# Yuki-Kumon/deepmatching_stereo_matching

Hardware: AMD Instinct MI355X
Metric: correlation-volume G-voxels/sec + ms/stereo-pair @1/8 GPU, 1024^2 d=128 (higher is better)
Workload: dtype u8->i32/f32/f64; 1 GPU; C3: 1024x1024 pair, 8x8 tiles of S=128, ws=5, full pyramid + sub-pixel + cal_map + stitch; tile=128, tiles_per_pair=64, window_size=5, pyramid_levels=full, parallelism=pairs sharded 1-way, streams=2, level_stream=False, stats_stream=False, pair_priority=normal, chain_levels=True

## Files before the change

deepmatching_stereo_matching_amd/_lib.py:

```python

import ctypes
import os
import re

import torch

HERE = os.path.dirname(os.path.abspath(__file__))
LIB_PATH = os.environ.get('DM_LIB_PATH') or os.path.join(HERE, 'libdmstereo.so')
HEADER = os.path.join(os.path.dirname(HERE), 'include', 'dmstereo.h')

DM_OK, DM_ERR_ARG, DM_ERR_SHAPE, DM_ERR_UNSUPPORTED, DM_ERR_HIP = 0, -1, -2, -3, -4
DM_VOLUME_F16, DM_VOLUME_MINMAX_KNOWN = 1, 2
DM_POW_F32, DM_POW_Q4, DM_POW_K, DM_POW_FULL, DM_POW_Q4G, DM_POW_KG = 0, 1, 2, 3, 4, 5
DM_TM_CCOEFF, DM_TM_CCOEFF_NORMED = 4, 5
METHODS = {'cv2.TM_CCOEFF_NORMED': DM_TM_CCOEFF_NORMED, 'cv2.TM_CCOEFF': DM_TM_CCOEFF}
CAL_MODES = {'elevation': 0, 'elevation2': 1, 'distance': 2}
DM_GS_FWD4, DM_GS_BWD4, DM_GS_BILAT = 0, 1, 2
DM_MERGE_LAST, DM_MERGE_CENTER, DM_MERGE_FEATHER, DM_MERGE_MEDIAN = 0, 1, 2, 3
MERGE_RULES = {'last': DM_MERGE_LAST, 'center': DM_MERGE_CENTER, 'feather': DM_MERGE_FEATHER,
               'median': DM_MERGE_MEDIAN}
DM_MERGE_MAX_CAND = 64
DM_BILAT_FILL, DM_BILAT_GUIDE_U8 = 1, 2
DM_MEDIAN_FILL = 1

# ... 2 lines not shown
    pass


class DmError(RuntimeError):
    pass


class DmTiles(ctypes.Structure):
    _fields_ = [('d_img1', ctypes.c_void_p), ('d_img2', ctypes.c_void_p),
                ('pitch1', ctypes.c_int32), ('pitch2', ctypes.c_int32),
                ('d_origins', ctypes.c_void_p), ('T', ctypes.c_int32),
                ('h0', ctypes.c_int32), ('w0', ctypes.c_int32),
                ('ws', ctypes.c_int32), ('method', ctypes.c_int32)]


_P = ctypes.c_void_p
_I = ctypes.c_int32
_TP = ctypes.POINTER(DmTiles)
SIGNATURES = {
    'dm_abi_version': ([], ctypes.c_int),
    'dm_last_error': ([], ctypes.c_char_p),
    'dm_build_config': ([], ctypes.c_char_p),
    'dm_stats_bytes': ([_TP], ctypes.c_size_t),
    'dm_corr_stats': ([_TP, _P, _P], ctypes.c_int),
    'dm_corr_level1': ([_TP, _P, _P, _P], ctypes.c_int),
    'dm_corr_level12': ([_TP, _P, _P, _P, _P], ctypes.c_int),
    'dm_corr_volume': ([_TP, _P, _P, _P], ctypes.c_int),
    'dm_corr_volume_f16': ([_TP, _P, _P, _P], ctypes.c_int),
    'dm_corr_volume_ex': ([_TP, _P, _I, _P, _P], ctypes.c_int),
    'dm_rectify_f16': ([_P, ctypes.c_size_t, _P, _P], ctypes.c_int),
    'dm_rectify': ([_P, ctypes.c_size_t, _P, _P], ctypes.c_int),
    'dm_rectify64': ([_P, ctypes.c_size_t, _P, _P], ctypes.c_int),
    'dm_pow14_variant': ([_I, _P, ctypes.c_size_t, _P, _P], ctypes.c_int),
    'dm_aggregate': ([_P, _I, _I, _I, _I, _P, _P], ctypes.c_int),
    'dm_match': ([_TP, _P, ctypes.POINTER(ctypes.c_void_p), _I, _I, _I, _I, _I, _I, _I, _I,
                  _P, _P, _P], ctypes.c_int),
    'dm_subpix_map': ([_P, _I, _I, _I, _I, _I, _P, _P], ctypes.c_int),
    'dm_subpix_map_tiles': ([_TP, _P, _I, _I, _P, _P], ctypes.c_int),
    'dm_sub_pix_cal': ([_P, _P, _I, _I, _I, ctypes.c_double, _P, _P], ctypes.c_int),
    'dm_cal_map': ([_P, _I, _I, _I, _I, _P, _P], ctypes.c_int),
    'dm_gs_schedule': ([_I, _I, _I, _I, _I, _I, _P, _P, ctypes.POINTER(ctypes.c_int32)], ctypes.c_int),
    'dm_image_threshold': ([_P, ctypes.c_size_t, ctypes.c_double, ctypes.c_double, _P, _P], ctypes.c_int),
    'dm_optimize_loop': ([_P, _P, _I, _I, _I, _I, _I, _I, _I, ctypes.c_double, _P, _P, _I, _P, _P, _I,
                          _P, _P, _P], ctypes.c_int),
    'dm_make_weight': ([_P, _I, _I, _I, _I, _I, ctypes.c_double, ctypes.c_double, _P, _P, _P], ctypes.c_int),
    'dm_opt_loop_bilateral': ([_P, _P, _P, _P, _I, _I, _I, _I, _I, _I, _I, _I, _P, _P, _I, _P, _P, _P],
                              ctypes.c_int),
    'dm_stitch': ([_P, _I, _I, _I, _I, _I, _I, ctypes.POINTER(ctypes.c_int32), _I, _P, _P, _P],
                  ctypes.c_int),
    'dm_seq_sum': ([_P, ctypes.c_int64, _P, _P], ctypes.c_int),
    'dm_fb_check': ([_P, _P, _I, _I, _I, ctypes.c_double, _P, _P, _P], ctypes.c_int),
    'dm_stitch_fb': ([_P, _P, _I, _I, _I, _I, _I, _I, ctypes.POINTER(ctypes.c_int32), _I, ctypes.c_double,
                      _P, _P, _P, _P], ctypes.c_int),
    'dm_stitch_merge': ([_P, _P, _I, _I, _I, _I, _I, _I, ctypes.POINTER(ctypes.c_int32), _I, ctypes.c_double,
                         _I, _I, _P, _P, _P, _P, _P, _P], ctypes.c_int),
    'dm_fill_bytes': ([_I, _I, _I], ctypes.c_size_t),
    'dm_fill_holes': ([_P, _I, _I, _I, _I, _P, _P, _P, _P], ctypes.c_int),
    'dm_speckle_bytes': ([_I, _I, _I], ctypes.c_size_t),
    'dm_filter_speckles': ([_P, _I, _I, _I, _I, ctypes.c_double, _P, _P, _P, _P, _P, _P], ctypes.c_int),
    'dm_bilateral_bytes': ([_I, _I, _I], ctypes.c_size_t),
    'dm_bilateral_filter': ([_P, _P, _I, _I, _I, _I, _I, ctypes.c_double, ctypes.c_double, _I, _I, _P, _P, _P, _P],
                            ctypes.c_int),
    'dm_median_bytes': ([_I, _I, _I], ctypes.c_size_t),
    'dm_median_filter': ([_P, _P, _I, _I, _I, _I, _I, _I, _I, _I, _P, _P, _P, _P], ctypes.c_int),
}

# ... 56 lines not shown
```

deepmatching_stereo_matching_amd/csrc/dm_kernels.hip:

```cpp
#include <hip/hip_runtime.h>

#include <stdarg.h>
#include <stdlib.h>
#include <stdio.h>
#include <string.h>

#include <type_traits>

#include "../../include/dmstereo.h"
#include "dm_pow.h"

__constant__ double c_pow_tab[DM_POW_NT * 3] = DM_POW_TAB_INIT;
__constant__ double c_pow_g[10] = DM_POW_G_INIT;
__constant__ double c_powf_c[DM_POWF_NT] = DM_POWF_C_INIT;
__constant__ double c_powf_p[DM_POWF_NT * 2] = DM_POWF_P_INIT;
__constant__ double c_powf_g[(1 - DM_POWF_EMIN) * 2] = DM_POWF_G_INIT;

#ifdef DM_TAIL_PRIO
#define DM_TAIL_ENTRY() __builtin_amdgcn_s_setprio(3)
#else
#define DM_TAIL_ENTRY() ((void)0)
#endif

__device__ __forceinline__ double pow14(double x)
// ... 1100 lines not shown

static int mfq_nw(const dm_tiles *b)
{
    const int G = b->w0 / 16;
    const bool g4 = b->ws * b->ws <= 25 && G % 4 == 0 && (G / 4 == 1 || G / 4 == 2 || G / 4 == 4);
    if (g4) return G / 4;
    return G / 2 < 8 ? G / 2 : 8;
}

static bool volume_ls_shape(const dm_tiles *b)
{
    return mf16_eligible(b) && b->ws <= 5 && (b->h0 % 4) == 0 && ((size_t)(b->h0 / 4) * (b->w0 / 4)) % 8 == 0;
}


#ifndef DM_S1
#define DM_S1 1
#endif
static bool strip_shape(const dm_tiles *b)
{
    if (!DM_S1 || !mf16_eligible(b) || b->ws > 5) return false;
    const int G = b->w0 / 16;
    return G % 4 == 0 && (G / 4 == 1 || G / 4 == 2 || G / 4 == 4);
}

#ifndef DM_S2
#define DM_S2 5
#endif
static bool strip2_shape(const dm_tiles *b)
{
    return strip_shape(b) && ((DM_S2 >> (b->w0 == 64 ? 0 : b->w0 == 128 ? 1 : 2)) & 1);
}

static size_t strip_bytes(const dm_tiles *b)
{
    const size_t rows = (size_t)b->T * (b->h0 / 2);
    return rows * (b->w0 / 32) * 1024 + rows * b->w0 * 16;
}

static void strip_views(const dm_tiles *b, void *d_stats, dm_v4i **Bs, dm_v4i **Ss)
{
    const size_t extra = mf16_extra_bytes(b);
    char *base = (char *)d_stats + align256(base_stats_bytes(b)) + align256(extra) +
                 (volume_ls_shape(b) ? align256(extra) : 0);
    *Bs = (dm_v4i *)base;
    *Ss = (dm_v4i *)(base + (size_t)b->T * (b->h0 / 2) * (b->w0 / 32) * 1024);
}

static void mfma_views2(const dm_tiles *b, void *d_stats, dm_v4i **Bw, int2 **QS)
{
    const int G = b->w0 / 16;
    char *base = (char *)d_stats + align256(base_stats_bytes(b)) + align256(mf16_extra_bytes(b));
    *Bw = (dm_v4i *)base;
    *QS = (int2 *)(base + (size_t)b->T * b->h0 * G * 1024);
}

static void mfma_views(const dm_tiles *b, void *d_stats, dm_v4i **Bw, int2 **QS)
{
    const int G = b->w0 / 16, KS = (b->ws * b->ws + 63) / 64;
    char *base = (char *)d_stats + align256(base_stats_bytes(b));
    *Bw = (dm_v4i *)base;
    *QS = (int2 *)(base + (size_t)b->T * b->h0 * G * KS * 1024);
}

static inline unsigned nblk(size_t n, unsigned bs)
{
// ... 156 lines not shown
static int launch_mfq_t(const dm_tiles *b, Stats s, const dm_v4i *Bw, const int2 *QS, double *L1, double *L2,
                        hipStream_t st, const dm_v4i *Bs, const dm_v4i *Ss)
{
    const int KS = (b->ws * b->ws + 63) / 64, NW = mfq_nw(b), GW = b->w0 / 16 / NW;
    const unsigned grid = (unsigned)(b->T * (b->h0 / 4) * (b->w0 / 4));
    const Geo gg = make_geo(b);
    constexpr bool CL = L2F;
    if (KS == 1 && GW == 4 && NW == 4) {
        constexpr int NBc = DM_C5_NB;
        const size_t bpt = (size_t)(b->h0 / 4) * (b->w0 / 4);
        if (bpt % NBc) return fail(DM_ERR_UNSUPPORTED, "cell blocks per tile not a multiple of %d (fill_ptab: a workgroup in one tile)", NBc);
        if (Bs && (DM_S2 & 4)) k_level12_strip<4, NBc, L2F, CL, 4><<<grid / NBc, 64 * 4 * NBc, 0, st>>>(gg, s, L1, L2, Bs, Ss);
        else if (Bs) k_level1_mfq<1, 4, 4 * NBc, 4, L2F, YF, NBc, CL, YF><<<grid / NBc, 64 * 4 * NBc, 0, st>>>(gg, s, Bw, QS, L1, L2, Bs, Ss);
        else k_level1_mfq<1, 4, 4 * NBc, 4, L2F, YF, NBc, CL><<<grid / NBc, 64 * 4 * NBc, 0, st>>>(gg, s, Bw, QS, L1, L2);
        HIP_TRY(hipGetLastError());
        return DM_OK;
    }
    if (KS == 1 && GW == 4 && NW == 1) {
        constexpr int NBc = DM_C2_NB;
        const size_t bpt = (size_t)(b->h0 / 4) * (b->w0 / 4);
        if (bpt % NBc) return fail(DM_ERR_UNSUPPORTED, "cell blocks per tile not a multiple of %d (fill_ptab: a workgroup in one tile)", NBc);
        if (Bs && (DM_S2 & 1)) k_level12_strip<1, NBc, L2F, CL, 4><<<grid / NBc, 64 * NBc, 0, st>>>(gg, s, L1, L2, Bs, Ss);
        else if (Bs) k_level1_mfq<1, 4, NBc, 4, L2F, YF, NBc, CL, YF><<<grid / NBc, 64 * NBc, 0, st>>>(gg, s, Bw, QS, L1, L2, Bs, Ss);
        else k_level1_mfq<1, 4, NBc, 4, L2F, YF, NBc, CL><<<grid / NBc, 64 * NBc, 0, st>>>(gg, s, Bw, QS, L1, L2);
        HIP_TRY(hipGetLastError());
        return DM_OK;
    }
    if (KS == 1 && GW == 4 && NW == 2) {
        constexpr int NBc = DM_C3_NB;
        const size_t bpt = (size_t)(b->h0 / 4) * (b->w0 / 4);
        if (bpt % NBc) return fail(DM_ERR_UNSUPPORTED, "cell blocks per tile not a multiple of %d (fill_ptab: a workgroup in one tile)", NBc);
        if (Bs && (DM_S2 & 2)) k_level12_strip<2, NBc, L2F, CL, DM_C3_MW><<<grid / NBc, 64 * 2 * NBc, 0, st>>>(gg, s, L1, L2, Bs, Ss);
        else if (prune_c3<L2F && YF>(gg, s, L1, L2, Bw, QS, Bs, Ss, grid / NBc, st)) {}
        else if (Bs) k_level1_mfq<1, 4, 2 * NBc, DM_C3_MINW, L2F, YF, NBc, CL, YF><<<grid / NBc, 64 * 2 * NBc, 0, st>>>(gg, s, Bw, QS, L1, L2, Bs, Ss);
        else k_level1_mfq<1, 4, 2 * NBc, 4, L2F, YF, NBc, CL><<<grid / NBc, 64 * 2 * NBc, 0, st>>>(gg, s, Bw, QS, L1, L2);
        HIP_TRY(hipGetLastError());
        return DM_OK;
    }
#define DM_MQ(KS_, GW_, NW_) if (KS == KS_ && GW == GW_ && NW == NW_) { k_level1_mfq<KS_, GW_, NW_, 5, L2F, YF><<<grid, 64 * NW_, 0, st>>>(gg, s, Bw, QS, L1, L2); HIP_TRY(hipGetLastError()); return DM_OK; }
    DM_MQ(1, 2, 1) DM_MQ(1, 2, 2) DM_MQ(1, 2, 4) DM_MQ(1, 2, 8)
    if constexpr (!YF) {
        DM_MQ(2, 2, 1) DM_MQ(2, 2, 2) DM_MQ(2, 2, 4) DM_MQ(2, 2, 8)
        DM_MQ(3, 2, 1) DM_MQ(3, 2, 2) DM_MQ(3, 2, 4) DM_MQ(3, 2, 8)
        DM_MQ(4, 2, 1) DM_MQ(4, 2, 2) DM_MQ(4, 2, 4) DM_MQ(4, 2, 8)
    }
#undef DM_MQ
    return fail(DM_ERR_UNSUPPORTED, "no column-split instance for KS=%d GW=%d NW=%d", KS, GW, NW);
}

template <bool L2F>
static int launch_mfq(const dm_tiles *b, void *d_stats, double *L1, double *L2, hipStream_t st)
{
    dm_v4i *Bw;
    int2 *QS;
    mfma_views(b, d_stats, &Bw, &QS);
    const Stats s = stats_view(d_stats, b->T, b->h0 * b->w0);
    dm_v4i *Bs = nullptr, *Ss = nullptr;
    if (strip_shape(b)) strip_views(b, d_stats, &Bs, &Ss);
    if (b->ws <= 5) return launch_mfq_t<L2F, true>(b, s, Bw, QS, L1, L2, st, Bs, Ss);
    return launch_mfq_t<L2F, false>(b, s, Bw, QS, L1, L2, st, nullptr, nullptr);
}

#ifndef DM_VL_H_TR
#define DM_VL_H_TR 2
#endif
#ifndef DM_VL_H_NT
// ... 99 lines not shown
    }
#define DM_VL(G_) if (G == G_) { k_volume_ls<G_, 8, true, OT><<<grid, 64 * 8, 0, st>>>(gg, s, Bw, QS, out, have_mm, Bs, Ss); HIP_TRY(hipGetLastError()); return DM_OK; }
    DM_VL(2) DM_VL(4) DM_VL(8) DM_VL(16)
#undef DM_VL
    return DM_ERR_UNSUPPORTED;
}

template <typename OT>
static int launch_volume_mfq(const dm_tiles *b, void *d_stats, const Stats &s, OT *out, hipStream_t st)
{
    dm_v4i *Bw;
    int2 *QS;
    mfma_views(b, d_stats, &Bw, &QS);
    const int KS = (b->ws * b->ws + 63) / 64, GW = b->w0 / 16 / mfq_nw(b);
    const size_t waves = (size_t)b->T * (b->h0 / 4) * (b->w0 / 4);
    const unsigned vgrid = (unsigned)((waves + 3) / 4);
    const bool lds = b->w0 <= 128;
    const Geo gg = make_geo(b);
#define DM_VQ(KS_, LS_) if (KS == KS_ && GW == 2 && lds == LS_) { k_volume_mfq<KS_, 2, false, true, LS_, OT><<<vgrid, 256, 0, st>>>(gg, s, Bw, QS, out); HIP_TRY(hipGetLastError()); return DM_OK; }
    DM_VQ(1, true) DM_VQ(1, false) DM_VQ(2, true) DM_VQ(2, false)
    DM_VQ(3, true) DM_VQ(3, false) DM_VQ(4, true) DM_VQ(4, false)
#undef DM_VQ
    return DM_ERR_UNSUPPORTED;
}

extern "C" {

int dm_abi_version(void) { return 110; }

#define DM_STR2(x) #x
#define DM_STR(x) DM_STR2(x)
const char *dm_build_config(void)
{
    return "S1=" DM_STR(DM_S1) " S2=" DM_STR(DM_S2) " PRUNE=" DM_STR(DM_PRUNE) " STRIP_WAVESYNC=" DM_STR(DM_STRIP_WAVESYNC) " VS1=" DM_STR(DM_VS1) " VS1_LDS=" DM_STR(DM_VS1_LDS) " XCD_MAP=" DM_STR(DM_XCD_MAP) " C2_NB=" DM_STR(DM_C2_NB) " C3_NB=" DM_STR(DM_C3_NB) " C3_MW=" DM_STR(DM_C3_MW) " C3_MINW=" DM_STR(DM_C3_MINW) " C5_NB=" DM_STR(DM_C5_NB)
           " VL_H_TR=" DM_STR(DM_VL_H_TR) " VL_H_NT=" DM_STR(DM_VL_H_NT) " VL_H_NW=" DM_STR(DM_VL_H_NW)
           " VL_H2_TR=" DM_STR(DM_VL_H2_TR) " VL_H2_NW=" DM_STR(DM_VL_H2_NW) " VL_F2_TR=" DM_STR(DM_VL_F2_TR)
           " VL_F2_MW=" DM_STR(DM_VL_F2_MW) " VL_HS_NW=" DM_STR(DM_VL_HS_NW) " VL_HS_TR=" DM_STR(DM_VL_HS_TR) " VL_F_NW=" DM_STR(DM_VL_F_NW)
           " VL_F_TR=" DM_STR(DM_VL_F_TR) " VL_F_MW=" DM_STR(DM_VL_F_MW) " VL_F_NT=" DM_STR(DM_VL_F_NT);
}

#if DM_CLOCK_STAMP
int dm_diag_clock_stamps(unsigned long long *host, int nwg)
{
    if (nwg < 0 || nwg > 65536) return fail(DM_ERR_ARG, "nwg %d outside 0 .. 65536", nwg);
    HIP_TRY(hipMemcpyFromSymbol(host, HIP_SYMBOL(dm_clock_stamps), (size_t)nwg * 4 * sizeof(unsigned long long)));
    return DM_OK;
}
#endif

const char *dm_last_error(void) { return g_err; }

size_t dm_stats_bytes(const dm_tiles *b)
{
    if (!b) return 0;
    size_t n = base_stats_bytes(b), extra = 0;
    if (b->ws >= 1 && b->ws <= 15 && b->T > 0 && b->h0 > 0 && b->w0 > 0 && mf16_eligible(b))
        extra = mf16_extra_bytes(b);
    if (!extra) return n;
    size_t tot = align256(n) + align256(extra);
    if (volume_ls_shape(b)) tot += align256(extra);
    if (strip_shape(b)) tot += strip_bytes(b);
    return tot;
}

int dm_corr_stats(const dm_tiles *b, void *d_stats, void *stream)
{
    int rc = check_tiles(b);
    if (rc) return rc;
    if (!d_stats) return fail(DM_ERR_ARG, "null stats workspace");
    const int P = b->h0 * b->w0;
    dim3 grid(nblk(P, 256), b->T);
    k_stats<<<grid, 256, 0, (hipStream_t)stream>>>(make_geo(b), stats_view(d_stats, b->T, P));
    HIP_TRY(hipGetLastError());
    const int var = level1_variant(b);
    if (var) {
        dm_v4i *Bw;
        int2 *QS;
        mfma_views(b, d_stats, &Bw, &QS);
        const int G = b->w0 / 16, KS = (b->ws * b->ws + 63) / 64;
        const size_t n = (size_t)b->T * b->h0 * G * 16;
        const int GW = G / mfq_nw(b);
        if (!strip2_shape(b)) {
            if (b->ws == 5) k_prep_windows16<5><<<nblk(n, 256), 256, 0, (hipStream_t)stream>>>(make_geo(b), G, GW, KS, Bw, QS);
            else k_prep_windows16<0><<<nblk(n, 256), 256, 0, (hipStream_t)stream>>>(make_geo(b), G, GW, KS, Bw, QS);
            HIP_TRY(hipGetLastError());
        }
        if (strip_shape(b)) {
            dm_v4i *Bs, *Ss;
            strip_views(b, d_stats, &Bs, &Ss);
            const size_t ns = (size_t)b->T * (b->h0 / 2) * b->w0;
            if (b->ws == 5) k_prep_strips<5><<<nblk(ns, 256), 256, 0, (hipStream_t)stream>>>(make_geo(b), Bs, Ss);
            else k_prep_strips<0><<<nblk(ns, 256), 256, 0, (hipStream_t)stream>>>(make_geo(b), Bs, Ss);
            HIP_TRY(hipGetLastError());
        }
    }
    return DM_OK;
}

int dm_corr_level1(const dm_tiles *b, void *d_stats, double *d_level1, void *stream)
{
    int rc = check_tiles(b);
    if (rc) return rc;
    if (!d_stats || !d_level1) return fail(DM_ERR_ARG, "null workspace / output");
    if ((b->h0 & 1) || (b->w0 & 1))
        return fail(DM_ERR_SHAPE, "could not broadcast: map sides %dx%d must be even (Correlation_map.py:96-103)", b->h0, b->w0);
    const int P = b->h0 * b->w0;
    Stats s = stats_view(d_stats, b->T, P);
    hipStream_t st = (hipStream_t)stream;
    const int var = level1_variant(b);
    if (var == 3) return launch_mfq<false>(b, d_stats, d_level1, nullptr, st);
    if (P > DM_GENERIC_MAX_P || k2_lds_bytes(b->h0, b->w0, b->ws) > 160 * 1024)
        return fail(DM_ERR_UNSUPPORTED, "tile too large for the generic level-1 kernel (P=%d)", P);
    switch (b->ws) {
    case 1: return launch_level1<1>(b, s, d_level1, st);
    case 3: return launch_level1<3>(b, s, d_level1, st);
// ... 84 lines not shown
{
    if (!d_in || !d_out) return fail(DM_ERR_ARG, "null pointer");
    if (n == 0) return DM_OK;
    k_rectify<_Float16><<<nblk(n, 256) > 8192 ? 8192 : nblk(n, 256), 256, 0, (hipStream_t)stream>>>(
        (const _Float16 *)d_in, n, d_out);
    HIP_TRY(hipGetLastError());
    return DM_OK;
}

int dm_rectify(const float *d_in, size_t n, double *d_out, void *stream)
{
    if (!d_in || !d_out) return fail(DM_ERR_ARG, "null pointer");
    if (n == 0) return DM_OK;
    k_rectify<float><<<nblk(n, 256) > 8192 ? 8192 : nblk(n, 256), 256, 0, (hipStream_t)stream>>>(d_in, n, d_out);
    HIP_TRY(hipGetLastError());
    return DM_OK;
}

int dm_pow14_variant(int32_t variant, const double *d_in, size_t n, double *d_out, void *stream)
{
    if ((!d_in || !d_out) && n) return fail(DM_ERR_ARG, "null input / output");
    if (!n) return DM_OK;
    const unsigned grid = nblk(n, 256) > 1024 ? 1024 : nblk(n, 256);
    hipStream_t st = (hipStream_t)stream;
    switch (variant) {
    case DM_POW_F32: k_pow_variant<DM_POW_F32><<<grid, 256, 0, st>>>(d_in, n, d_out); break;
    case DM_POW_Q4: k_pow_variant<DM_POW_Q4><<<grid, 256, 0, st>>>(d_in, n, d_out); break;
    case DM_POW_K: k_pow_variant<DM_POW_K><<<grid, 256, 0, st>>>(d_in, n, d_out); break;
    case DM_POW_Q4G: k_pow_variant<DM_POW_Q4G><<<grid, 256, 0, st>>>(d_in, n, d_out); break;
    case DM_POW_KG: k_pow_variant<DM_POW_KG><<<grid, 256, 0, st>>>(d_in, n, d_out); break;
    case DM_POW_FULL: k_pow_variant<DM_POW_FULL><<<grid, 256, 0, st>>>(d_in, n, d_out); break;
    default: return fail(DM_ERR_ARG, "unknown pow14 variant %d", variant);
    }
    HIP_TRY(hipGetLastError());
    return DM_OK;
}

int dm_rectify64(const double *d_in, size_t n, double *d_out, void *stream)
{
    if (!d_in || !d_out) return fail(DM_ERR_ARG, "null pointer");
    if (n == 0) return DM_OK;
    k_rectify<double><<<nblk(n, 256) > 8192 ? 8192 : nblk(n, 256), 256, 0, (hipStream_t)stream>>>(d_in, n, d_out);
    HIP_TRY(hipGetLastError());
    return DM_OK;
}

int dm_aggregate(const double *d_in, int32_t T, int32_t h, int32_t w, int32_t rectify, double *d_out,
                 void *stream)
{
    if (!d_in || !d_out || T < 1 || h < 1 || w < 1) return fail(DM_ERR_ARG, "bad aggregate arguments");
    if ((h & 1) || (w & 1))
        return fail(DM_ERR_SHAPE, "could not broadcast: map side %d must halve (Correlation_map.py:96-103)", (h & 1) ? h : w);
    const int W2 = w / 2, h2 = h / 2;
    const char *ag = getenv("DM_AGGREGATE");
    if (W2 >= 16 && 4 * W2 <= 256 && !(ag && ag[0] == '0')) {
        const int BR = AGG_LDS_DOUBLES / (4 * W2) < h2 ? AGG_LDS_DOUBLES / (4 * W2) : h2;
        const size_t nwg = (size_t)T * h2 * W2 * ((h2 + BR - 1) / BR);
        if (nwg <= 0x7fffffff) {
            const bool vec = ((uintptr_t)d_in & 15) == 0 && (W2 == 16 || W2 == 32 || W2 == 64);
            const size_t lds = (size_t)4 * BR * W2 * sizeof(double);
            if (vec) k_aggregate_rows<true><<<(unsigned)nwg, 4 * W2, lds, (hipStream_t)stream>>>(d_in, T, h, w, BR, rectify, d_out);
            else k_aggregate_rows<false><<<(unsigned)nwg, 4 * W2, lds, (hipStream_t)stream>>>(d_in, T, h, w, BR, rectify, d_out);
            HIP_TRY(hipGetLastError());
            return DM_OK;
        }
    }
// ... 194 lines not shown
```

deepmatching_stereo_matching_amd/csrc/dm_mfma.h:

```cpp
#pragma once

typedef int dm_v4i __attribute__((ext_vector_type(4)));
typedef int dm_v2i __attribute__((ext_vector_type(2)));


template <int WSC>
__global__ void k_prep_windows16(Geo g, int G, int GW, int KS, dm_v4i *Bw, int2 *QS)
{
    DM_TAIL_ENTRY();
    const size_t idx = blockIdx.x * (size_t)blockDim.x + threadIdx.x;
    const size_t total = (size_t)g.T * g.h0 * G * 16;
    if (idx >= total) return;
    const int c = (int)(idx % 16);
    const int tau = (int)((idx / 16) % G);
    const int q0 = (int)((idx / (16 * (size_t)G)) % g.h0);
    const int t = (int)(idx / (16 * (size_t)G * g.h0));
    const int q1 = 16 * GW * (tau / GW) + GW * c + (tau % GW);
    const int ws = WSC ? WSC : g.ws, n = ws * ws;
    const uint8_t *base = g.img2 + (size_t)(g.org[2 * t] + q0) * g.pitch2 + g.org[2 * t + 1] + q1;
    int pix[WSC ? WSC * WSC : 1];
    if constexpr (WSC != 0) {
#pragma unroll
        for (int k = 0; k < WSC * WSC; ++k) pix[k] = (int)base[(size_t)(k / WSC) * g.pitch2 + (k % WSC)] - 128;
    }
    auto px = [&](int k) -> int {
        if constexpr (WSC != 0) return pix[k];
        else return (int)base[(size_t)(k / ws) * g.pitch2 + (k % ws)] - 128;
    };
    int s = 0, s2 = 0;
#pragma unroll
    for (int k = 0; k < n; ++k) {
        const int b = px(k);
        s += b; s2 += b * b;
    }
    const long long dI = (long long)n * s2 - (long long)s * s;
    float bq;
    if (g.method == DM_TM_CCOEFF) bq = 1.0f;
    else bq = dI == 0 ? 0.0f : (float)(1.0 / sqrt((double)dI));
    const int qx = __float_as_int((float)-s), qy = __float_as_int(bq);
    QS[idx] = make_int2(qx, qy);
    const size_t tile = idx / 16;
    const bool spread = KS == 1 && n <= 32;
    for (int ks = 0; ks < KS; ++ks)
        for (int hq = 0; hq < 4; ++hq) {
            int w[4] = {0, 0, 0, 0};
            if (spread) {
                for (int j = 0; j < 8; ++j) {
                    const int k = 8 * hq + j;
                    const int val = k < n ? px(k) : 0;
                    w[j >> 2] |= (val & 0xFF) << (8 * (j & 3));
                }
                w[2] = qx;
                w[3] = qy;
            } else {
                for (int j = 0; j < 16; ++j) {
                    const int k = 64 * ks + 16 * hq + j;
                    const int val = k < n ? px(k) : 0;
                    w[j >> 2] |= (val & 0xFF) << (8 * (j & 3));
                }
            }
            dm_v4i o;
            o.x = w[0]; o.y = w[1]; o.z = w[2]; o.w = w[3];
            Bw[(tile * KS + ks) * 64 + c + 16 * hq] = o;
        }
}

typedef int dm_v16i __attribute__((ext_vector_type(16)));
typedef float dm_f2 __attribute__((ext_vector_type(2)));

__device__ __forceinline__ int2 window_qs(int s, int s2, int n, int method)
{
    const long long dI = (long long)n * s2 - (long long)s * s;
    float bq;
    if (method == DM_TM_CCOEFF) bq = 1.0f;
    else bq = dI == 0 ? 0.0f : (float)(1.0 / sqrt((double)dI));
    return make_int2(__float_as_int((float)-s), __float_as_int(bq));
}

__device__ __forceinline__ __amdgpu_buffer_rsrc_t tile_rsrc(const uint8_t *img, int pitch, const Geo &g, int t)
{
    const int ro = __builtin_amdgcn_readfirstlane(g.org[2 * t]), co = __builtin_amdgcn_readfirstlane(g.org[2 * t + 1]);
    return __builtin_amdgcn_make_buffer_rsrc((void *)(img + (size_t)ro * pitch + co), 0, 0x7fffffff, 0x00020000);
}

template <int WSC>
__global__ void k_prep_strips(Geo g, dm_v4i *Bs, dm_v4i *Ss)
// ... 256 lines not shown

__device__ __forceinline__ void lds_dma16(__amdgpu_buffer_rsrc_t r, unsigned lds_byte, unsigned voff, unsigned soff)
{
    unsigned keep;
    asm volatile("s_mov_b32 %0, m0\n\ts_mov_b32 m0, %1\n\ts_nop 0\n\tbuffer_load_dwordx4 %2, %3, %4 offen lds\n\ts_mov_b32 m0, %0"
                 : "=&s"(keep) : "s"(lds_byte), "v"(voff), "s"(r), "s"(soff) : "memory");
}

__device__ __forceinline__ dm_f2 pk_fma_clamp01(dm_f2 a, dm_f2 b, dm_f2 c)
{
    dm_f2 r;
    asm("v_pk_fma_f32 %0, %1, %2, %3 clamp" : "=v"(r) : "v"(a), "v"(b), "v"(c));
    return r;
}
__device__ __forceinline__ bool cell_flat(float4 den)
{
    return den.x == 0.0f || den.y == 0.0f || den.z == 0.0f || den.w == 0.0f;
}
__device__ __forceinline__ bool block_has_flat(const float4 (&cst)[4][6])
{
    return cell_flat(cst[0][4]) || cell_flat(cst[1][4]) || cell_flat(cst[2][4]) || cell_flat(cst[3][4]);
}

template <bool H, typename T, int OFF = 0>
struct XchOwn {
    __attribute__((aligned(16))) T v;
    __device__ T &get(PowLds &) { return v; }
};
template <typename T, int OFF>
struct XchOwn<true, T, OFF> {
    __device__ T &get(PowLds &p) { return *reinterpret_cast<T *>((char *)&p.g32[128] + OFF); }
};

template <int KS, int GW, int NW, int MINW, bool L2F, bool YF, int NB = 1, bool CL = false, bool S1 = false>
__global__ __launch_bounds__(64 * NW, MINW) void k_level1_mfq(Geo g, Stats s, const dm_v4i *__restrict__ Bw,
                                                        const int2 *__restrict__ QS, double *L1, double *L2,
                                                        const dm_v4i *__restrict__ Bs = nullptr,
                                                        const dm_v4i *__restrict__ Ss = nullptr)
{
    DM_CLOCK_STAMP_HERE
    constexpr bool EQ = KS == 1 && YF;
    static_assert(NW % NB == 0, "blocks split the waves evenly");
    static_assert(!CL || L2F, "clamp-bit normalisation: NaN cells are restored at the level-2 / level-1 stores");
    constexpr int NWc = NW / NB;
    constexpr int XS = NWc > 1 ? NWc + 1 : 1;
    constexpr int XW = NWc > 1 ? NWc : 1;
    __shared__ PowLds plds;
    struct Xch {
        float xch[NB][2][2][XS][4][4];
        double stash[L2F ? NW : 1][64];
        double xch2[NB][2][XW][4];
    };
    struct Red {
        float red[NB][2][NWc][16];
    };
    constexpr bool HOLE = sizeof(Xch) <= G32_HOLE;
    constexpr bool HOLE_R = HOLE && sizeof(Xch) + sizeof(Red) <= G32_HOLE;
    __shared__ XchOwn<HOLE, Xch> xown;
    __shared__ XchOwn<HOLE_R, Red, (int)sizeof(Xch)> rown;
    Xch &X = xown.get(plds);
    auto &xch = X.xch;
    auto &stash = X.stash;
    auto &xch2 = X.xch2;
    auto &red = rown.get(plds).red;
    __shared__ float4 cst[NB][4][6];
    constexpr bool LATE = L2F && DM_LATE;
    constexpr int L2V = 4 * GW, L2B = 64 / L2V;
    constexpr int RB = 64 / (4 * L2V);
    __shared__ double stash2[L2F && GW == 2 ? NW : 1][L2F && GW == 2 ? 64 : 1];
    const int tid = threadIdx.x;
    pow_lds_fill(plds, tid, 64 * NW, HOLE);
    if (NWc > 1 && tid < 64 * NB)
        (&xch[tid >> 6][0][0][0][0][0])[((tid & 63) >> 4) * XS * 16 + (tid & 15)] = -INFINITY;
    __shared__ __attribute__((aligned(16))) unsigned ptab[S1 ? NB : 1][16][16];
    if constexpr (S1) {
        const int nbj_ = (g.w0 / 2) / 2, bpt_ = ((g.h0 / 2) / 2) * nbj_;
        if (g.ws == 5) fill_ptab<S1 ? NB : 1, 64 * NW, 5>(ptab, g, tid, bpt_, nbj_);
        else fill_ptab<S1 ? NB : 1, 64 * NW, 0>(ptab, g, tid, bpt_, nbj_);
    }
    __syncthreads();

    constexpr int G = GW * NWc;
    const int lane = tid & 63, wave = __builtin_amdgcn_readfirstlane(tid >> 6);
    const int sb = NB > 1 ? wave / NWc : 0, wc = NB > 1 ? wave % NWc : wave;
    const int c = lane & 15, grp = lane >> 4;
    const int h0 = g.h0, w0 = g.w0, n = g.ws * g.ws, P = h0 * w0;
    const int w1 = w0 / 2, P1 = (h0 / 2) * w1;
    const int nbj = w1 / 2, bpt = ((h0 / 2) / 2) * nbj;
    const int blk = wg_logical() * NB + sb;
    const int t = blk / bpt;
    const int I0 = 2 * ((blk % bpt) / nbj), J0 = 2 * ((blk % bpt) % nbj);
    const size_t tb = (size_t)t * P;
    const int ro = g.org[2 * t], co = g.org[2 * t + 1];

    dm_v4i A[KS];
    const int Ic = I0 + (grp >> 1), Jc = J0 + (grp & 1);
    int sTr[4];
    float sTf[4];
    auto init_a16 = [&]() {
        if constexpr (S1) {
            const dm_v2i tp = *(const dm_v2i *)&ptab[sb][c][2 * grp];
            A[0] = dm_v4i{tp.x, tp.y, 0, 0};
        } else {
            build_a<KS>(A, g, t, I0, J0, c, grp);
        }
#pragma unroll
        for (int r = 0; r < 4; ++r) {
            const int p = (2 * Ic + (r >> 1)) * w0 + 2 * Jc + (r & 1);
            sTr[r] = s.sT[tb + p];
            sTf[r] = (float)sTr[r];
        }
    };
    if constexpr (!S1) init_a16();
    const int ab = YF ? DM_YBIAS : 0;
    const dm_v4i acc0 = {ab, ab, ab, ab};
    const unsigned mant = mant_mask_vgpr();
    const dm_v4i *Bt = Bw + ((size_t)t * h0 * G + wc * GW) * KS * 64;
    const int2 *Qt = QS + ((size_t)t * h0 * G + wc * GW) * 16;

    struct RowFrag {
        dm_v4i b[GW][KS];
        int2 q[GW];
    };
    const __amdgpu_buffer_rsrc_t rB = __builtin_amdgcn_make_buffer_rsrc((void *)Bt, 0, 0x7fffffff, 0x00020000);
    const __amdgpu_buffer_rsrc_t rQ = __builtin_amdgcn_make_buffer_rsrc((void *)Qt, 0, 0x7fffffff, 0x00020000);
    const unsigned voB = (unsigned)lane * 16u, voQ = (unsigned)c * 8u;
    auto load_row = [&](RowFrag &f, int q0) {
#pragma unroll
        for (int tw = 0; tw < GW; ++tw) {
            const unsigned ti = (unsigned)q0 * G + tw;
#pragma unroll
            for (int ks = 0; ks < KS; ++ks)
                f.b[tw][ks] = __builtin_amdgcn_raw_buffer_load_b128(rB, voB, (ti * KS + ks) * 1024u, 0);
            if constexpr (!EQ) {
                const dm_v2i qv = __builtin_amdgcn_raw_buffer_load_b64(rQ, voQ, ti * 128u, 0);
                f.q[tw] = make_int2(qv.x, qv.y);
            }
        }
    };

    float mn[4], mx[4];
#pragma unroll
    for (int r = 0; r < 4; ++r) { mn[r] = INFINITY; mx[r] = -INFINITY; }
    auto minmax_row = [&](const RowFrag &f) {
#pragma unroll
        for (int tw = 0; tw < GW; ++tw) {
            const dm_v4i acc = mfma_tile<KS, EQ>(A, f.b[tw], acc0);
            float y[4];
            y_of_acc<YF>(acc, sTr, sTf, EQ ? qs_of_frag(f.b[tw][0]) : qs_pair(f.q[tw]), n, y);
#pragma unroll
            for (int r = 0; r < 4; ++r) {
                mn[r] = fminf(mn[r], y[r]);
                mx[r] = fmaxf(mx[r], y[r]);
            }
        }
    };
    RowFrag fa, fb;
    if constexpr (S1) {
        static_assert(YF && KS == 1 && GW == 4, "strip sweep: packed y, one 64-window column group per wave");
        const int c32 = lane & 31, hs = lane >> 5;
// ... 91 lines not shown
        const int p = (2 * Ic + (r >> 1)) * w0 + 2 * Jc + (r & 1);
        const float ap = s.aP[tb + p];
        float a = red[sb][0][0][4 * grp + r], b = red[sb][1][0][4 * grp + r];
#pragma unroll
        for (int w = 1; w < NWc; ++w) { a = fminf(a, red[sb][0][w][4 * grp + r]); b = fmaxf(b, red[sb][1][w][4 * grp + r]); }
        const float rmn = r_of_y(a, ap, g.method), rmx = r_of_y(b, ap, g.method);
        const float den = __fsub_rn(rmx, rmn);
        const bool cc = g.method == DM_TM_CCOEFF;
        float *f = (float *)&cst[sb][grp][0];
        f[0 * 4 + r] = ap;
        f[1 * 4 + r] = cc ? -INFINITY : (ap == 0.0f ? 1.0f : -1.0f);
        f[2 * 4 + r] = cc ? INFINITY : 1.0f;
        f[3 * 4 + r] = rmn;
        f[4 * 4 + r] = den;
        f[5 * 4 + r] = __frcp_rn(den);
        s.rmn[tb + p] = rmn;
        s.rmx[tb + p] = rmx;
    }
    __syncthreads();

    const bool bflat = CL && __builtin_amdgcn_readfirstlane((int)block_has_flat(cst[sb])) != 0;
    const bool cflat = CL && L1 && cell_flat(cst[sb][grp][4]);
    constexpr int M = GW / 2;
    constexpr int M2 = M >= 2 ? M / 2 : 1;
    float Cprev[M][4];
    double Racc2[M2], Cprev2[M2], l1p[M];
    double *Lrow = L1 ? L1 + ((size_t)t * P1 + (size_t)Ic * w1 + Jc) * P1 + 8 * GW * wc : nullptr;
    const int w2 = w0 / 4, P2 = (h0 / 4) * w2;
    double *L2row = L2F ? L2 + ((size_t)t * P2 + (size_t)(I0 / 2) * w2 + J0 / 2) * P2 : nullptr;

    auto pool_cols = [&](const RowFrag &f, float (&Cm)[M][4], float (&last)[4]) {
#pragma unroll
        for (int tw = 0; tw < GW; ++tw) {
            const dm_v4i acc = mfma_tile<KS, EQ>(A, f.b[tw], acc0);
            float y[4];
            y_of_acc<YF>(acc, sTr, sTf, EQ ? qs_of_frag(f.b[tw][0]) : qs_pair(f.q[tw]), n, y);
#pragma unroll
            for (int r = 0; r < 4; ++r) {
                if ((tw & 1) == 0) Cm[tw / 2][r] = tw == 0 ? y[r] : fmaxf(last[r], y[r]);
                else Cm[tw / 2][r] = fmaxf(Cm[tw / 2][r], y[r]);
                last[r] = y[r];
            }
        }
    };

    auto level2_row = [&](int u, const double (&l1p)[M]) {
        const double lft = __shfl(l1p[M - 1], lane - 1);
        const double left = c != 0 ? lft : (wc == 0 ? l1p[0] : xch2[sb][u & 1][wc - 1][grp]);
        double Cq[M2];
        if constexpr (M == 1) {
            const double right = __shfl(l1p[0], lane + 1);
            Cq[0] = cellmax_d(cellmax_d(left, l1p[0]), right);
        } else {
#pragma unroll
            for (int j = 0; j < M2; ++j)
                Cq[j] = cellmax_d(cellmax_d(j == 0 ? left : l1p[2 * j - 1], l1p[2 * j]), l1p[2 * j + 1]);
        }
        if ((u & 1) == 0) {
#pragma unroll
            for (int j = 0; j < M2; ++j) Racc2[j] = u == 0 ? Cq[j] : cellmax_d(Cprev2[j], Cq[j]);
        } else {
            const int u2 = u >> 1, slot = u2 % L2B;
            if constexpr (M == 1) {
                const double R2 = cellmax_d(Racc2[0], Cq[0]);
                Cprev2[0] = Cq[0];
                const int rb = u2 % RB;
                if ((c & 1) == 0) stash2[wave][rb * 4 * L2V + grp * L2V + c / 2] = R2;
                if (rb == RB - 1 || u2 == h0 / 4 - 1) {
                    __builtin_amdgcn_fence(__ATOMIC_RELEASE, "wavefront");
// ... 711 lines not shown
```

include/dmstereo.h:

```cpp
#ifndef DMSTEREO_H
#define DMSTEREO_H

#include <stddef.h>
#include <stdint.h>

#ifdef __cplusplus
extern "C" {
#endif

enum dm_status {
    DM_OK = 0,
    DM_ERR_ARG = -1,
    DM_ERR_SHAPE = -2,
    DM_ERR_UNSUPPORTED = -3,
    DM_ERR_HIP = -4
};

enum dm_method {
    DM_TM_CCOEFF = 4,
    DM_TM_CCOEFF_NORMED = 5
};

enum dm_cal_mode {
    DM_CAL_ELEVATION = 0,
// ... 9 lines not shown
    int32_t T;
    int32_t h0, w0;
    int32_t ws;
    int32_t method;
} dm_tiles;

size_t dm_stats_bytes(const dm_tiles *b);

int dm_corr_stats(const dm_tiles *b, void *d_stats, void *stream);

int dm_corr_level1(const dm_tiles *b, void *d_stats, double *d_level1, void *stream);

int dm_corr_level12(const dm_tiles *b, void *d_stats, double *d_level1, double *d_level2, void *stream);

int dm_corr_volume(const dm_tiles *b, void *d_stats, float *d_l0, void *stream);

int dm_corr_volume_f16(const dm_tiles *b, void *d_stats, uint16_t *d_l0, void *stream);

enum {
    DM_VOLUME_F16 = 1,
    DM_VOLUME_MINMAX_KNOWN = 2
};

int dm_corr_volume_ex(const dm_tiles *b, void *d_stats, int32_t flags, void *d_l0, void *stream);

int dm_rectify_f16(const uint16_t *d_in, size_t n, double *d_out, void *stream);

int dm_rectify(const float *d_in, size_t n, double *d_out, void *stream);

int dm_rectify64(const double *d_in, size_t n, double *d_out, void *stream);

enum dm_pow_variant { DM_POW_F32 = 0, DM_POW_Q4 = 1, DM_POW_K = 2, DM_POW_FULL = 3, DM_POW_Q4G = 4, DM_POW_KG = 5 };
int dm_pow14_variant(int32_t variant, const double *d_in, size_t n, double *d_out, void *stream);

int dm_aggregate(const double *d_in, int32_t T, int32_t h, int32_t w, int32_t rectify,
                 double *d_out, void *stream);

int dm_match(const dm_tiles *b, const void *d_stats, const double *const *d_levels,
             int32_t nlev, int32_t T, int32_t h0, int32_t w0, int32_t sub_pix,
             int32_t filter_window, int32_t filter_num, int32_t filter_mode,
             double *d_scratch, double *d_out, void *stream);

int dm_subpix_map(const double *d_level0, int32_t T, int32_t h0, int32_t w0, int32_t hm, int32_t wm,
                  double *d_map, void *stream);

int dm_subpix_map_tiles(const dm_tiles *b, const void *d_stats, int32_t hm, int32_t wm, double *d_map,
                        void *stream);

int dm_sub_pix_cal(const double *d_arr, const double *d_score, int32_t h, int32_t w,
                   int32_t direction, double ratio, double *d_out, void *stream);

int dm_cal_map(const double *d_map, int32_t T, int32_t h, int32_t w, int32_t mode,
               double *d_out, void *stream);

int dm_stitch(const double *d_match, int32_t n0, int32_t n1, int32_t h0, int32_t w0,
              int32_t stride0, int32_t stride1, const int32_t *modes, int32_t nmodes,
              double *d_dmap, double *d_score, void *stream);


int dm_fb_check(const double *d_fwd, const double *d_bwd, int32_t T, int32_t h, int32_t w,
                double tol, double *d_err, double *d_masked, void *stream);

int dm_stitch_fb(const double *d_fwd, const double *d_bwd, int32_t n0, int32_t n1, int32_t h0,
                 int32_t w0, int32_t stride0, int32_t stride1, const int32_t *modes,
                 int32_t nmodes, double tol, double *d_dmap, double *d_score, double *d_err,
                 void *stream);
// ... 83 lines not shown
```

Before: 2439 Gvox/s.

## Compute level-1 correlation numerator with f16 MFMA folding mean terms into padding

For 128-wide strip tiles, the level-1 correlation numerator now runs on the f16 16x16x32 MFMA. The patch and window sums are folded into spare K slots, split into low and high parts, so the mean subtraction happens inside the matrix op. This replaces the int8 MFMA plus scalar y_of_acc correction with one f16 MFMA and a multiply by a precomputed per-window float scale. The window prep writes the f16 fragments and a separate float scale array. This cuts per-tile ALU work, at the cost of f16 rounding risk and a changed buffer layout, and adds debug and query entry points.

```diff
diff --git a/deepmatching_stereo_matching_amd/_lib.py b/deepmatching_stereo_matching_amd/_lib.py
--- a/deepmatching_stereo_matching_amd/_lib.py
+++ b/deepmatching_stereo_matching_amd/_lib.py
@@ -58,6 +58,8 @@
     'dm_rectify': ([_P, ctypes.c_size_t, _P, _P], ctypes.c_int),
     'dm_rectify64': ([_P, ctypes.c_size_t, _P, _P], ctypes.c_int),
     'dm_pow14_variant': ([_I, _P, ctypes.c_size_t, _P, _P], ctypes.c_int),
+    'dm_debug_num_tile_f16': ([_P, _P, _I, _P, _P], ctypes.c_int),
+    'dm_level_num_f16': ([_TP], ctypes.c_int),
     'dm_aggregate': ([_P, _I, _I, _I, _I, _P, _P], ctypes.c_int),
     'dm_match': ([_TP, _P, ctypes.POINTER(ctypes.c_void_p), _I, _I, _I, _I, _I, _I, _I, _I,
                   _P, _P, _P], ctypes.c_int),
diff --git a/deepmatching_stereo_matching_amd/csrc/dm_kernels.hip b/deepmatching_stereo_matching_amd/csrc/dm_kernels.hip
--- a/deepmatching_stereo_matching_amd/csrc/dm_kernels.hip
+++ b/deepmatching_stereo_matching_amd/csrc/dm_kernels.hip
@@ -1156,6 +1156,14 @@
     return strip_shape(b) && ((DM_S2 >> (b->w0 == 64 ? 0 : b->w0 == 128 ? 1 : 2)) & 1);
 }
 
+#ifndef DM_F16Y
+#define DM_F16Y 1
+#endif
+static bool f16y_shape(const dm_tiles *b)
+{
+    return DM_F16Y && !DM_PRUNE && strip_shape(b) && !strip2_shape(b) && b->w0 == 128;
+}
+
 static size_t strip_bytes(const dm_tiles *b)
 {
     const size_t rows = (size_t)b->T * (b->h0 / 2);
@@ -1378,6 +1386,9 @@
         if (bpt % NBc) return fail(DM_ERR_UNSUPPORTED, "cell blocks per tile not a multiple of %d (fill_ptab: a workgroup in one tile)", NBc);
         if (Bs && (DM_S2 & 2)) k_level12_strip<2, NBc, L2F, CL, DM_C3_MW><<<grid / NBc, 64 * 2 * NBc, 0, st>>>(gg, s, L1, L2, Bs, Ss);
         else if (prune_c3<L2F && YF>(gg, s, L1, L2, Bw, QS, Bs, Ss, grid / NBc, st)) {}
+        else if (f16y_shape(b)) {
+            if constexpr (YF) k_level1_mfq<1, 4, 2 * NBc, DM_C3_MINW, L2F, YF, NBc, CL, YF, YF><<<grid / NBc, 64 * 2 * NBc, 0, st>>>(gg, s, Bw, QS, L1, L2, Bs, Ss);
+        }
         else if (Bs) k_level1_mfq<1, 4, 2 * NBc, DM_C3_MINW, L2F, YF, NBc, CL, YF><<<grid / NBc, 64 * 2 * NBc, 0, st>>>(gg, s, Bw, QS, L1, L2, Bs, Ss);
         else k_level1_mfq<1, 4, 2 * NBc, 4, L2F, YF, NBc, CL><<<grid / NBc, 64 * 2 * NBc, 0, st>>>(gg, s, Bw, QS, L1, L2);
         HIP_TRY(hipGetLastError());
@@ -1543,7 +1554,7 @@
 #define DM_STR(x) DM_STR2(x)
 const char *dm_build_config(void)
 {
-    return "S1=" DM_STR(DM_S1) " S2=" DM_STR(DM_S2) " PRUNE=" DM_STR(DM_PRUNE) " STRIP_WAVESYNC=" DM_STR(DM_STRIP_WAVESYNC) " VS1=" DM_STR(DM_VS1) " VS1_LDS=" DM_STR(DM_VS1_LDS) " XCD_MAP=" DM_STR(DM_XCD_MAP) " C2_NB=" DM_STR(DM_C2_NB) " C3_NB=" DM_STR(DM_C3_NB) " C3_MW=" DM_STR(DM_C3_MW) " C3_MINW=" DM_STR(DM_C3_MINW) " C5_NB=" DM_STR(DM_C5_NB)
+    return "S1=" DM_STR(DM_S1) " F16Y=" DM_STR(DM_F16Y) " S2=" DM_STR(DM_S2) " PRUNE=" DM_STR(DM_PRUNE) " STRIP_WAVESYNC=" DM_STR(DM_STRIP_WAVESYNC) " VS1=" DM_STR(DM_VS1) " VS1_LDS=" DM_STR(DM_VS1_LDS) " XCD_MAP=" DM_STR(DM_XCD_MAP) " C2_NB=" DM_STR(DM_C2_NB) " C3_NB=" DM_STR(DM_C3_NB) " C3_MW=" DM_STR(DM_C3_MW) " C3_MINW=" DM_STR(DM_C3_MINW) " C5_NB=" DM_STR(DM_C5_NB)
            " VL_H_TR=" DM_STR(DM_VL_H_TR) " VL_H_NT=" DM_STR(DM_VL_H_NT) " VL_H_NW=" DM_STR(DM_VL_H_NW)
            " VL_H2_TR=" DM_STR(DM_VL_H2_TR) " VL_H2_NW=" DM_STR(DM_VL_H2_NW) " VL_F2_TR=" DM_STR(DM_VL_F2_TR)
            " VL_F2_MW=" DM_STR(DM_VL_F2_MW) " VL_HS_NW=" DM_STR(DM_VL_HS_NW) " VL_HS_TR=" DM_STR(DM_VL_HS_TR) " VL_F_NW=" DM_STR(DM_VL_F_NW)
@@ -1572,6 +1583,12 @@
     if (volume_ls_shape(b)) tot += align256(extra);
     if (strip_shape(b)) tot += strip_bytes(b);
     return tot;
+}
+
+int dm_level_num_f16(const dm_tiles *b)
+{
+    if (!b || b->ws < 1 || b->ws > 15 || b->T <= 0 || b->h0 <= 0 || b->w0 <= 0) return 0;
+    return f16y_shape(b) ? 1 : 0;
 }
 
 int dm_corr_stats(const dm_tiles *b, void *d_stats, void *stream)
@@ -1591,7 +1608,11 @@
         const int G = b->w0 / 16, KS = (b->ws * b->ws + 63) / 64;
         const size_t n = (size_t)b->T * b->h0 * G * 16;
         const int GW = G / mfq_nw(b);
-        if (!strip2_shape(b)) {
+        if (f16y_shape(b)) {
+            if (b->ws == 5) k_prep_windows16<5, true><<<nblk(n, 256), 256, 0, (hipStream_t)stream>>>(make_geo(b), G, GW, KS, Bw, QS);
+            else k_prep_windows16<0, true><<<nblk(n, 256), 256, 0, (hipStream_t)stream>>>(make_geo(b), G, GW, KS, Bw, QS);
+            HIP_TRY(hipGetLastError());
+        } else if (!strip2_shape(b)) {
             if (b->ws == 5) k_prep_windows16<5><<<nblk(n, 256), 256, 0, (hipStream_t)stream>>>(make_geo(b), G, GW, KS, Bw, QS);
             else k_prep_windows16<0><<<nblk(n, 256), 256, 0, (hipStream_t)stream>>>(make_geo(b), G, GW, KS, Bw, QS);
             HIP_TRY(hipGetLastError());
@@ -1742,6 +1763,16 @@
     case DM_POW_FULL: k_pow_variant<DM_POW_FULL><<<grid, 256, 0, st>>>(d_in, n, d_out); break;
     default: return fail(DM_ERR_ARG, "unknown pow14 variant %d", variant);
     }
+    HIP_TRY(hipGetLastError());
+    return DM_OK;
+}
+
+int dm_debug_num_tile_f16(const uint8_t *d_patch_taps, const uint8_t *d_window_taps, int32_t ws,
+                          float *d_num, void *stream)
+{
+    if (!d_patch_taps || !d_window_taps || !d_num) return fail(DM_ERR_ARG, "null taps / output");
+    if (ws != 1 && ws != 3 && ws != 5) return fail(DM_ERR_UNSUPPORTED, "window side %d: the f16 num tile takes 1, 3 or 5", ws);
+    k_debug_num_tile_f16<<<1, 64, 0, (hipStream_t)stream>>>(d_patch_taps, d_window_taps, ws, d_num);
     HIP_TRY(hipGetLastError());
     return DM_OK;
 }
diff --git a/deepmatching_stereo_matching_amd/csrc/dm_mfma.h b/deepmatching_stereo_matching_amd/csrc/dm_mfma.h
--- a/deepmatching_stereo_matching_amd/csrc/dm_mfma.h
+++ b/deepmatching_stereo_matching_amd/csrc/dm_mfma.h
@@ -3,8 +3,65 @@
 typedef int dm_v4i __attribute__((ext_vector_type(4)));
 typedef int dm_v2i __attribute__((ext_vector_type(2)));
 
-
-template <int WSC>
+#ifndef DM_ABL_F16Y
+#define DM_ABL_F16Y 0
+#endif
+#define DM_ABL_F16_FINITE ((int)0xBFFFBFFF)
+
+typedef _Float16 dm_v8h __attribute__((ext_vector_type(8)));
+typedef float dm_v4f __attribute__((ext_vector_type(4)));
+
+template <bool WIN>
+__device__ __forceinline__ int f16_slot(int k, int n, int ws, int tap, int s)
+{
+    if (k < n) return ws * tap;
+    const int j = k - n;
+    if (j >= 4) return 0;
+    const int lo = s & 63, hi = s - lo;
+    if (WIN) return (j & 1) ? -lo : -hi;
+    return (j & 2) ? lo : hi;
+}
+
+template <bool WIN, typename F>
+__device__ __forceinline__ dm_v4i f16_frag(F tap, int s, int n, int ws, int hq)
+{
+    int w[4];
+#pragma unroll
+    for (int j = 0; j < 8; j += 2) {
+        unsigned h[2];
+#pragma unroll
+        for (int e = 0; e < 2; ++e) {
+            const int k = 8 * hq + j + e;
+            const _Float16 v = (_Float16)f16_slot<WIN>(k, n, ws, k < n ? tap(k) : 0, s);
+            h[e] = __builtin_bit_cast(unsigned short, v);
+        }
+        w[j >> 1] = (int)(h[0] | (h[1] << 16));
+    }
+    return dm_v4i{w[0], w[1], w[2], w[3]};
+}
+
+__device__ __forceinline__ dm_v4f num_tile_f16(const dm_v4i &a, const dm_v4i &b)
+{
+    return __builtin_amdgcn_mfma_f32_16x16x32_f16(__builtin_bit_cast(dm_v8h, a), __builtin_bit_cast(dm_v8h, b),
+                                                  dm_v4f{0.0f, 0.0f, 0.0f, 0.0f}, 0, 0, 0);
+}
+
+__global__ __launch_bounds__(64) void k_debug_num_tile_f16(const uint8_t *__restrict__ pt,
+                                                           const uint8_t *__restrict__ wt, int ws, float *out)
+{
+    const int lane = threadIdx.x & 63, c = lane & 15, hq = lane >> 4, n = ws * ws;
+    auto tp = [&](int k) { return (int)pt[c * n + k] - 128; };
+    auto tw = [&](int k) { return (int)wt[c * n + k] - 128; };
+    int sT = 0, sI = 0;
+    for (int k = 0; k < n; ++k) { sT += tp(k); sI += tw(k); }
+    const dm_v4f d = num_tile_f16(f16_frag<false>(tp, sT, n, ws, hq), f16_frag<true>(tw, sI, n, ws, hq));
+#pragma unroll
+    for (int r = 0; r < 4; ++r) out[16 * (4 * hq + r) + c] = d[r];
+}
+
+
+
+template <int WSC, bool F16 = false>
 __global__ void k_prep_windows16(Geo g, int G, int GW, int KS, dm_v4i *Bw, int2 *QS)
 {
     DM_TAIL_ENTRY();
@@ -38,8 +95,14 @@
     if (g.method == DM_TM_CCOEFF) bq = 1.0f;
     else bq = dI == 0 ? 0.0f : (float)(1.0 / sqrt((double)dI));
     const int qx = __float_as_int((float)-s), qy = __float_as_int(bq);
+    const size_t tile = idx / 16;
+    if constexpr (F16) {
+        ((float *)QS)[((size_t)t * g.h0 + q0) * g.w0 + q1] = bq;
+#pragma unroll
+        for (int hq = 0; hq < 4; ++hq) Bw[tile * 64 + c + 16 * hq] = f16_frag<true>(px, s, n, ws, hq);
+        return;
+    }
     QS[idx] = make_int2(qx, qy);
-    const size_t tile = idx / 16;
     const bool spread = KS == 1 && n <= 32;
     for (int ks = 0; ks < KS; ++ks)
         for (int hq = 0; hq < 4; ++hq) {
@@ -52,6 +115,9 @@
                 }
                 w[2] = qx;
                 w[3] = qy;
+#if DM_ABL_F16Y
+                w[0] &= DM_ABL_F16_FINITE; w[1] &= DM_ABL_F16_FINITE; w[3] &= (int)0xFFFFBFFF;
+#endif
             } else {
                 for (int j = 0; j < 16; ++j) {
                     const int k = 64 * ks + 16 * hq + j;
@@ -374,13 +440,15 @@
     __device__ T &get(PowLds &p) { return *reinterpret_cast<T *>((char *)&p.g32[128] + OFF); }
 };
 
-template <int KS, int GW, int NW, int MINW, bool L2F, bool YF, int NB = 1, bool CL = false, bool S1 = false>
+template <int KS, int GW, int NW, int MINW, bool L2F, bool YF, int NB = 1, bool CL = false, bool S1 = false,
+          bool F16 = false>
 __global__ __launch_bounds__(64 * NW, MINW) void k_level1_mfq(Geo g, Stats s, const dm_v4i *__restrict__ Bw,
                                                         const int2 *__restrict__ QS, double *L1, double *L2,
                                                         const dm_v4i *__restrict__ Bs = nullptr,
                                                         const dm_v4i *__restrict__ Ss = nullptr)
 {
     DM_CLOCK_STAMP_HERE
+    static_assert(!F16 || (S1 && KS == 1 && GW == 4 && YF), "f16 num: strip sweep 1, one 16-byte b_q load per lane and row");
     constexpr bool EQ = KS == 1 && YF;
     static_assert(NW % NB == 0, "blocks split the waves evenly");
     static_assert(!CL || L2F, "clamp-bit normalisation: NaN cells are restored at the level-2 / level-1 stores");
@@ -440,9 +508,23 @@
     int sTr[4];
     float sTf[4];
     auto init_a16 = [&]() {
+        if constexpr (F16) {
+            const dm_v2i tp = *(const dm_v2i *)&ptab[sb][c][2 * grp];
+            const int cl = c >> 2, ch = c & 3;
+            const int pa = (2 * (I0 + (cl >> 1)) + (ch >> 1)) * w0 + 2 * (J0 + (cl & 1)) + (ch & 1);
+            auto tap = [&](int k) {
+                const int j = k - 8 * grp;
+                return (int)(signed char)(((unsigned)(j < 4 ? tp.x : tp.y)) >> (8 * (j & 3)));
+            };
+            A[0] = f16_frag<false>(tap, s.sT[tb + pa], n, g.ws, grp);
+            return;
+        }
         if constexpr (S1) {
             const dm_v2i tp = *(const dm_v2i *)&ptab[sb][c][2 * grp];
             A[0] = dm_v4i{tp.x, tp.y, 0, 0};
+#if DM_ABL_F16Y
+            A[0].x &= DM_ABL_F16_FINITE; A[0].y &= DM_ABL_F16_FINITE;
+#endif
         } else {
             build_a<KS>(A, g, t, I0, J0, c, grp);
         }
@@ -463,11 +545,15 @@
     struct RowFrag {
         dm_v4i b[GW][KS];
         int2 q[GW];
+        dm_v4f bq;
     };
     const __amdgpu_buffer_rsrc_t rB = __builtin_amdgcn_make_buffer_rsrc((void *)Bt, 0, 0x7fffffff, 0x00020000);
-    const __amdgpu_buffer_rsrc_t rQ = __builtin_amdgcn_make_buffer_rsrc((void *)Qt, 0, 0x7fffffff, 0x00020000);
-    const unsigned voB = (unsigned)lane * 16u, voQ = (unsigned)c * 8u;
+    const void *Qb = F16 ? (const void *)((const float *)QS + (size_t)t * P + 16 * GW * wc) : (const void *)Qt;
+    const __amdgpu_buffer_rsrc_t rQ = __builtin_amdgcn_make_buffer_rsrc((void *)Qb, 0, 0x7fffffff, 0x00020000);
+    const unsigned voB = (unsigned)lane * 16u, voQ = F16 ? (unsigned)c * 16u : (unsigned)c * 8u;
     auto load_row = [&](RowFrag &f, int q0) {
+        if constexpr (F16)
+            f.bq = __builtin_bit_cast(dm_v4f, __builtin_amdgcn_raw_buffer_load_b128(rQ, voQ, (unsigned)(q0 * w0) * 4u, 0));
 #pragma unroll
         for (int tw = 0; tw < GW; ++tw) {
             const unsigned ti = (unsigned)q0 * G + tw;
@@ -625,9 +711,27 @@
     auto pool_cols = [&](const RowFrag &f, float (&Cm)[M][4], float (&last)[4]) {
 #pragma unroll
         for (int tw = 0; tw < GW; ++tw) {
-            const dm_v4i acc = mfma_tile<KS, EQ>(A, f.b[tw], acc0);
             float y[4];
-            y_of_acc<YF>(acc, sTr, sTf, EQ ? qs_of_frag(f.b[tw][0]) : qs_pair(f.q[tw]), n, y);
+            if constexpr (F16) {
+                const dm_v4f d = num_tile_f16(A[0], f.b[tw][0]);
+                const dm_f2 q2 = tw < 2 ? dm_f2{f.bq[0], f.bq[1]} : dm_f2{f.bq[2], f.bq[3]};
+                const dm_f2 bb = (tw & 1) ? __builtin_shufflevector(q2, q2, 1, 1) : __builtin_shufflevector(q2, q2, 0, 0);
+                const dm_f2 y01 = dm_f2{d[0], d[1]} * bb, y23 = dm_f2{d[2], d[3]} * bb;
+                y[0] = y01.x; y[1] = y01.y; y[2] = y23.x; y[3] = y23.y;
+            } else
+#if DM_ABL_F16Y
+            if constexpr (S1 && EQ) {
+                const dm_v4f d = num_tile_f16(A[0], f.b[tw][0]);
+                const dm_f2 q2 = qs_of_frag(f.b[tw][0]);
+                const dm_f2 bb = __builtin_shufflevector(q2, q2, 1, 1);
+                const dm_f2 y01 = dm_f2{d[0], d[1]} * bb, y23 = dm_f2{d[2], d[3]} * bb;
+                y[0] = y01.x; y[1] = y01.y; y[2] = y23.x; y[3] = y23.y;
+            } else
+#endif
+            {
+                const dm_v4i acc = mfma_tile<KS, EQ>(A, f.b[tw], acc0);
+                y_of_acc<YF>(acc, sTr, sTf, EQ ? qs_of_frag(f.b[tw][0]) : qs_pair(f.q[tw]), n, y);
+            }
 #pragma unroll
             for (int r = 0; r < 4; ++r) {
                 if ((tw & 1) == 0) Cm[tw / 2][r] = tw == 0 ? y[r] : fmaxf(last[r], y[r]);
diff --git a/include/dmstereo.h b/include/dmstereo.h
--- a/include/dmstereo.h
+++ b/include/dmstereo.h
@@ -65,6 +65,11 @@
 
 enum dm_pow_variant { DM_POW_F32 = 0, DM_POW_Q4 = 1, DM_POW_K = 2, DM_POW_FULL = 3, DM_POW_Q4G = 4, DM_POW_KG = 5 };
 int dm_pow14_variant(int32_t variant, const double *d_in, size_t n, double *d_out, void *stream);
+
+int dm_debug_num_tile_f16(const uint8_t *d_patch_taps, const uint8_t *d_window_taps, int32_t ws,
+                          float *d_num, void *stream);
+
+int dm_level_num_f16(const dm_tiles *b);
 
 int dm_aggregate(const double *d_in, int32_t T, int32_t h, int32_t w, int32_t rectify,
                  double *d_out, void *stream);
```

Result: faster. 2530 Gvox/s, median of 6 (+3.7%).
